# serviceberry3/weiner_slamit_v2

Measured on AMD Instinct MI355X. Metric: frames/sec ORB extract+match @640x480x8lvl, higher is better.
Workload: dtype u8; 1 GPU; BASELINE configs[1]: 640x480 8-level ORB extract (1000 features, FAST 20/7) + brute-force 256-bit Hamming best/second match vs the stream's previous frame; 256 independent streams per GPU per step; distinct_frame_pairs_per_gpu=16, parallelism=streams sharded over 1 GPU(s), no data-path collective

## Files before the change

### weiner_slamit_v2_amd/csrc/octree_table.h

```cpp
#ifndef SLAMIT_OCTREE_TABLE_H
#define SLAMIT_OCTREE_TABLE_H
#include <stdint.h>

#if defined(__HIPCC__)
#define OCT_HD __host__ __device__ __forceinline__
#else
#define OCT_HD static inline
#endif

#define OCT_FD_MAX 4

struct Box16 { short x0, y0, x1, y1; };

OCT_HD int box_quadrant(const Box16& b, int x, int y, int* mx, int* my) {
    int midx = b.x0 + ((b.x1 - b.x0 + 1) >> 1);
    int midy = b.y0 + ((b.y1 - b.y0 + 1) >> 1);
    *mx = midx; *my = midy;
    return (x < midx ? 0 : 1) + (y < midy ? 0 : 2);
}
OCT_HD Box16 child_box(const Box16& b, int q) {
    int midx = b.x0 + ((b.x1 - b.x0 + 1) >> 1);
    int midy = b.y0 + ((b.y1 - b.y0 + 1) >> 1);
    Box16 c;
    c.x0 = (q & 1) ? midx : b.x0; c.x1 = (q & 1) ? b.x1 : midx;
    c.y0 = (q & 2) ? midy : b.y0; c.y1 = (q & 2) ? b.y1 : midy;
    return c;
}

// ... 9 lines not shown
}
OCT_HD unsigned oct_rank_key(int cnt, int pos) { return ((unsigned)cnt << 12) | (unsigned)(4095 - pos); }

OCT_HD int oct_key_root(int x, float hX, int nIni) {
    const int r = (int)((float)x / hX);
    return r < nIni - 1 ? r : nIni - 1;
}
OCT_HD int oct_key_path(Box16 b, int x, int y, int FD) {
    int path = 0;
    for (int d = 0; d < FD; ++d) {
        int mx, my;
        const int q = box_quadrant(b, x, y, &mx, &my);
        b = child_box(b, q);
        path = path * 4 + q;
    }
    return path;
}

OCT_HD unsigned long long oct_pick_key(unsigned response, unsigned order) {
    return ((unsigned long long)response << 32) | (0xFFFFFFFFu - order);
}
OCT_HD unsigned oct_pick_response(unsigned long long k) { return (unsigned)(k >> 32); }
OCT_HD unsigned oct_pick_order(unsigned long long k) { return 0xFFFFFFFFu - (unsigned)k; }

OCT_HD int oct_code(int root, int depth, int path) { return (root << 16) | (depth << 12) | path; }
OCT_HD int oct_code_root(int c) { return c >> 16; }
OCT_HD int oct_code_depth(int c) { return (c >> 12) & 15; }
OCT_HD int oct_code_path(int c) { return c & 4095; }
OCT_HD int oct_code_child(int c, int q) { return oct_code(oct_code_root(c), oct_code_depth(c) + 1, 4 * oct_code_path(c) + q); }
OCT_HD int oct_child_slot(int c, int q, int HS) {
    return oct_code_root(c) * HS + oct_depth_off(oct_code_depth(c) + 1) + 4 * oct_code_path(c) + q;
}
OCT_HD int oct_node_slot(int c, int HS) { return oct_code_root(c) * HS + oct_depth_off(oct_code_depth(c)) + oct_code_path(c); }

OCT_HD bool oct_node_leaves_table(int cnt, int code, int FD) { return cnt > 1 && oct_code_depth(code) >= FD; }

OCT_HD void oct_table_sum_up(int* tab, int FD) {
    for (int d = FD - 1; d >= 1; --d)
        for (int p = 0; p < (1 << (2 * d)); ++p) {
            const int* c = &tab[oct_depth_off(d + 1) + 4 * p];
            tab[oct_depth_off(d) + p] = (c[0] + c[1]) + (c[2] + c[3]);
        }
}

#define OCT_PATH_LEFT 0x100
OCT_HD int oct_path_word(int passes, bool left) { return (passes & 0xFF) | (left ? OCT_PATH_LEFT : 0); }
// ... 93 lines not shown
```

### weiner_slamit_v2_amd/csrc/orb_api.hip

```cpp
#include <hip/hip_runtime.h>
#include <math.h>
#include <stdio.h>
#include <stdlib.h>
#include <string.h>

#include <algorithm>
#include <vector>

#include "../../include/slamit.h"
#include "orb_plan.h"
#include "slamit_internal.h"

hipError_t orbk_upload_pattern(hipStream_t st);
void orbk_resize(hipStream_t st, const uint8_t* src, int sw, int sh, size_t sstride, size_t sframe,
                 uint8_t* dst, int dw, int dh, size_t dstride, size_t dframe, const int* xofs,
                 const short* ialpha, const int* yofs, const short* ibeta, int nframes);
void orbk_resize_rows4(hipStream_t st, const uint8_t* src, size_t sstride, size_t sframe, int sh, uint8_t* dst, int dw, int dh,
                       size_t dstride, size_t dframe, const uint32_t* d_col, const uint32_t* d_row, int nframes);
void orbk_resize_rows8(hipStream_t st, const uint8_t* src, size_t sstride, size_t sframe, int sh, uint8_t* dst, int dw, int dh,
                       size_t dstride, size_t dframe, const uint32_t* d_col8, const uint32_t* d_row, int nframes);
hipError_t orbk_pyramid_bands_prepare(int smem_bytes);
void orbk_pyramid_bands(hipStream_t st, const BandTab& tab, const uint8_t* d_tables, const BandRows* d_rows, int first, int last, int nbands,
                        const uint8_t* src, size_t sstride, size_t sframe, int sh, uint8_t* pyr, size_t pyr_frame, int tile0, int smem, int nframes);
hipError_t orbk_pyramid_prepare(int smem_bytes);
void orbk_pyramid(hipStream_t st, const OrbLevel* levels, int nlevels, const PyrBox* boxes, const PyrTabs* tabs,
                  int nregions, const uint8_t* img0, size_t img0_stride, size_t img0_frame, uint8_t* pyr, int bufA_bytes,
                  int smem_bytes, int nframes, int l_first, int l_last);
hipError_t orbk_fast_prepare(int max_wcell, int max_hcell);
void orbk_fast(hipStream_t st, const FastTab& tab, int nlevels, const uint32_t* d_cells, int cells_per_frame, const uint8_t* img0,
               size_t img0_stride, size_t img0_frame, const uint8_t* pyr, unsigned long long* cand,
               size_t cand_frame_stride, int* cand_count, int iniTh, int minTh, int max_wcell, int max_hcell, int nframes);
hipError_t orbk_octree_prepare(int node_cap, int key_cap);
void orbk_octree(hipStream_t st, const OrbLevel* levels, int nlevels, const unsigned long long* cand,
                 size_t cand_frame_stride, int* cand_count, uint32_t* ws_xy, uint16_t* ws_node,
                 OrbLevelKp* lkp, size_t kp_frame_stride, int* kp_count, int node_cap, int key_cap, int nframes,
                 int level_override);
void orbk_ic_angle(hipStream_t st, const OrbLevel* levels, int nlevels, const uint8_t* img0, size_t img0_stride,
                   size_t img0_frame, const uint8_t* pyr, OrbLevelKp* lkp, size_t kp_frame_stride,
                   const int* kp_count, const KpBlockTab& tab, int nframes);
void orbk_blur_stream(hipStream_t st, const OrbLevel* levels, const uint32_t* d_inner, int n_inner, const uint32_t* d_edge, int n_edge,
                      const uint8_t* img0, size_t img0_stride, size_t img0_frame, const uint8_t* pyr, uint8_t* blur, int nframes);
void orbk_blur(hipStream_t st, const OrbLevel* levels, const uint32_t* d_tiles, int total_tiles, const uint8_t* img0,
               size_t img0_stride, size_t img0_frame, const uint8_t* pyr, uint8_t* blur, int nframes);
void orbk_describe(hipStream_t st, const OrbLevel* levels, int nlevels, const uint8_t* blur,
                   const OrbLevelKp* lkp, size_t kp_frame_stride, const int* kp_count, slamit_kp* out_kps,
                   uint8_t* out_desc, int out_cap, int* out_n, const KpBlockTab& tab, int nframes);
void orbk_pad(hipStream_t st, const uint8_t* src, int w, int h, size_t sstride, uint8_t* dst);
void orbk_decode_candidates(hipStream_t st, const OrbLevel* levels, int level, const unsigned long long* K, int n,
                            unsigned long long* order_out, int* xys);

namespace {

inline size_t round_up(size_t v, size_t a) { return (v + a - 1) / a * a; }

}

#define ORB_BLUR_SPLIT 1

struct slamit_orb {
// ... 233 lines not shown
            const OrbLevel& D = P.levels[l];
            const uint8_t* src = l == 1 ? d_gray : h->d_pyr + S.plane_off;
            size_t sstride = l == 1 ? stride : (size_t)S.stride;
            size_t sframe = l == 1 ? frame_stride : P.pyr_frame_total;
            const OrbResizeTabs& T = P.rs[l];
            orbk_resize(st, src, S.w, S.h, sstride, sframe, h->d_pyr + D.plane_off, D.w, D.h, (size_t)D.stride,
                        P.pyr_frame_total, dtab<int>(h, T.xofs_off), dtab<short>(h, T.ialpha_off), dtab<int>(h, T.yofs_off),
                        dtab<short>(h, T.ibeta_off), nframes);
        }
    }
    prof_mark(h, st, ST_RESIZE, false);
    prof_mark(h, st, ST_FAST, true);
    orbk_fast(st, P.fast, nl, dtab<uint32_t>(h, P.cells_off), (int)(P.cells.size() / 4), d_gray, stride, frame_stride, h->d_pyr, h->d_cand,
              P.cand_frame_stride, cand_count, h->p.ini_th_fast, h->p.min_th_fast, P.max_wcell, P.max_hcell, nframes);
    prof_mark(h, st, ST_FAST, false);
    if (side) {
        HIP_TRY(hipEventRecord(h->ev_pyr, st));
        HIP_TRY(hipStreamWaitEvent(h->stream_b, h->ev_pyr, 0));
        launch_blur(h->stream_b, early_done + 1, nl);
        HIP_TRY(hipEventRecord(h->ev_blur, h->stream_b));
    }
    prof_mark(h, st, ST_OCTREE, true);
    orbk_octree(st, h->d_levels, nl, h->d_cand, P.cand_frame_stride, cand_count, h->d_ws_xy, h->d_ws_node, h->d_lkp,
                P.kp_frame_stride, kp_count, P.node_cap, P.oct_key_cap, nframes, -1);
    prof_mark(h, st, ST_OCTREE, false);
    prof_mark(h, st, ST_ANGLE, true);
    orbk_ic_angle(st, h->d_levels, nl, d_gray, stride, frame_stride, h->d_pyr, h->d_lkp, P.kp_frame_stride, kp_count,
                  P.ic_blocks, nframes);
    prof_mark(h, st, ST_ANGLE, false);
    if (side) {
        HIP_TRY(hipStreamWaitEvent(st, h->ev_blur, 0));
    } else {
        prof_mark(h, st, ST_BLUR, true);
        launch_blur(st, 0, nl);
        prof_mark(h, st, ST_BLUR, false);
    }
    prof_mark(h, st, ST_DESCRIBE, true);
    orbk_describe(st, h->d_levels, nl, h->d_blur, h->d_lkp, P.kp_frame_stride, kp_count, d_kps, d_desc, cap, d_n_out,
                  P.desc_blocks, nframes);
    prof_mark(h, st, ST_DESCRIBE, false);
    ++h->prof_call;
    HIP_TRY(hipGetLastError());
    h->counters_clean = true;
    h->last_img0 = d_gray; h->last_stride = stride; h->last_frame = frame_stride; h->last_nframes = nframes;
    return SLAMIT_OK;
}

// ... 151 lines not shown
```

### weiner_slamit_v2_amd/csrc/orb_kernels.hip

```cpp
#include <hip/hip_runtime.h>
#include <stdint.h>

#include <algorithm>

#include "blur_window.h"
#include "octree_table.h"
#include "orb_types.h"
#include "slamit_math.h"
#include "wave_ops.h"
#include "../../include/slamit.h"
#include "../../include/slamit_orb_pattern.h"

#define WAVE 64

__global__ __launch_bounds__(256) void resize_level_kernel(
    const uint8_t* __restrict__ src, int sw, int sh, size_t sstride, size_t sframe,
    uint8_t* __restrict__ dst, int dw, int dh, size_t dstride, size_t dframe,
    const int* __restrict__ xofs, const short* __restrict__ ialpha,
    const int* __restrict__ yofs, const short* __restrict__ ibeta) {
    const int x4 = (blockIdx.x * 64 + (threadIdx.x & 63)) * 4;
    const int y = blockIdx.y * 4 + (threadIdx.x >> 6);
    const int f = blockIdx.z;
    if (x4 >= dw || y >= dh) return;
    const uint8_t* S = src + (size_t)f * sframe;
// ... 1081 lines not shown
    __syncthreads();
    for (int i = tid; i < n; i += NT) {
        unsigned long long b = best[i];
        unsigned order = 0xFFFFFFFFu - (unsigned)b;
        int lx = order & 63, ly = (order >> 6) & 63, cell = order >> 12;
        int ci = cell / L.nCols, cj = cell - ci * L.nCols;
        OrbLevelKp kp;
        kp.x = (int16_t)(cj * L.wCell + lx + ORB_MIN_BORDER);
        kp.y = (int16_t)(ci * L.hCell + ly + ORB_MIN_BORDER);
        kp.response = (float)(unsigned)(b >> 32);
        kp.angle = 0.f; kp.cs = 1.f; kp.sn = 0.f;
        if (i < L.kp_cap) OUT[i] = kp;
    }
    if (tid == 0) *kp_count_out = min(n, L.kp_cap);
#ifdef OCT_DIAG
    OD_STAMP(5);
    if (tid == 0) {
        const int w = blockIdx.y * gridDim.x + blockIdx.x;
        if (w < 4096) { unsigned long long* o = g_oct_ph + 8 * w; for (int k = 0; k < 6; ++k) o[k] = od_ph[k]; o[6] = ((unsigned long long)od_pass << 32) | (unsigned)n_keys; o[7] = od_rt0; o[5] = __builtin_amdgcn_s_memrealtime(); }
    }
#endif
}

template <int NT>
__device__ __forceinline__ bool octree_table_path(
    const OrbLevel& L, const unsigned long long* __restrict__ K, int n_keys, OrbLevelKp* __restrict__ OUT,
    int* __restrict__ kp_count_out, unsigned char* smem, int cap, unsigned long long* bin_best, int FD, int* s_vars, int* passes_out) {
    const int tid = threadIdx.x, lane = tid & 63;
    const int nIni = L.nIni, N = L.quota;
    const int HS = oct_table_ints(FD), NB = oct_bins(FD), leaf0 = oct_depth_off(FD);
    int* const hist = reinterpret_cast<int*>(smem);
    int* const ncode0 = reinterpret_cast<int*>(smem + (size_t)8 * cap);
    unsigned long long* const nbest = reinterpret_cast<unsigned long long*>(smem + (size_t)16 * cap);
    int* const cnt0 = reinterpret_cast<int*>(smem + (size_t)24 * cap);
    int* const elist = cnt0 + 2 * cap;
    unsigned* const ekey = reinterpret_cast<unsigned*>(elist + cap);
    int* const scanbuf = elist + 4 * cap;
    int* const rankv = scanbuf + 5 * cap;
    int* const sorted = rankv + cap;
    Box16* const rootbox = reinterpret_cast<Box16*>(scanbuf);
    OD_DECL;

    if (tid < nIni) { Box16 b; b.x0 = (short)L.rootUL[tid]; b.y0 = 0; b.x1 = (short)L.rootUR[tid]; b.y1 = (short)L.boxH; rootbox[tid] = b; }
    for (int e = tid; e < nIni * HS; e += NT) hist[e] = 0;
    for (int e = tid; e < nIni * NB; e += NT) bin_best[e] = 0ull;
    __syncthreads();
    {
        const int nCols = L.nCols, wCell = L.wCell, hCell = L.hCell;
        const unsigned inv_cols = 0xFFFFFFFFu / (unsigned)nCols + 1u;
        const float hX = L.hX;
        for (int kb4 = 0; kb4 < n_keys; kb4 += 4 * NT) {
            unsigned long long c4[4];
#pragma unroll
            for (int j = 0; j < 4; ++j) c4[j] = K[min(kb4 + j * NT + tid, n_keys - 1)];
#pragma unroll
            for (int j = 0; j < 4; ++j) {
                const int kb = kb4 + j * NT;
                if (kb >= n_keys) break;
                const bool valid = kb + tid < n_keys;
                const unsigned order = (unsigned)c4[j];
                const int lx = order & 63, ly = (order >> 6) & 63, cell = order >> 12;
                const int ci = (int)__umulhi((unsigned)cell, inv_cols), cj = cell - ci * nCols;
                const int x = cj * wCell + lx, y = ci * hCell + ly;
                const int r = oct_key_root(x, hX, nIni);
                const int path = oct_key_path(rootbox[r], x, y, FD);
                const int bin = valid ? r * NB + path : -1;
                const int prev = __shfl_up(bin, 1);
                const bool head = lane == 0 || bin != prev;
                const unsigned long long heads = __ballot(head);
                const unsigned long long rest = (heads >> lane) >> 1;
                const int last = rest ? lane + (int)__builtin_ctzll(rest) : 63;
                unsigned long long pk = valid ? oct_pick_key((unsigned)(c4[j] >> 32), order) : 0ull;
#pragma unroll
                for (int s = 1; s < 64; s <<= 1) {
                    const unsigned long long o = __shfl_down(pk, s);
                    pk = (lane + s <= last && o > pk) ? o : pk;
                }
                if (head && bin >= 0) {
                    atomicAdd(&hist[r * HS + leaf0 + path], last - lane + 1);
                    atomicMax(&bin_best[bin], pk);
                }
            }
        }
    }
    __syncthreads();
    OD_STAMP(0);

    if (tid < 64) {
        for (int d = FD - 1; d >= 1; --d) {
            const int per = 1 << (2 * d), off = oct_depth_off(d), offc = oct_depth_off(d + 1);
            for (int e = lane; e < nIni * per; e += 64) {
                const int r = e >> (2 * d), pth = e & (per - 1);
                const int* c = &hist[r * HS + offc + 4 * pth];
                hist[r * HS + off + pth] = (c[0] + c[1]) + (c[2] + c[3]);
            }
            wave_mem_sync();
        }
        if (lane == 0) {
            int m = 0;
            for (int i = 0; i < nIni; ++i) {
                const int c = (hist[i * HS] + hist[i * HS + 1]) + (hist[i * HS + 2] + hist[i * HS + 3]);
                if (c > 0) { cnt0[m] = c; ncode0[m] = oct_code(i, 0, 0); ++m; }
            }
            s_vars[0] = m;
        }
        wave_mem_sync();
// ... 95 lines not shown
            else if (!careful && n + nToExpand * 3 > N) careful = true;
        }
        if (!left) {
            int* const rootlab = scanbuf;
            int* const lab = scanbuf + ORB_MAX_ROOTS;
            for (int e = lane; e < nIni * HS; e += 64) lab[e] = -1;
            if (lane < ORB_MAX_ROOTS) rootlab[lane] = -1;
            for (int i = lane; i < n; i += 64) nbest[i] = 0ull;
            wave_mem_sync();
            for (int i = lane; i < n; i += 64) {
                const int c = ncode0[cur * cap + i];
                if (oct_code_depth(c) == 0) rootlab[oct_code_root(c)] = i;
                else lab[oct_node_slot(c, HS)] = i;
            }
        }
        if (lane == 0) { s_vars[0] = n; s_vars[2] = passes; s_vars[3] = left; }
    }
    __syncthreads();
    OD_STAMP(1);
    *passes_out = s_vars[2];
    if (s_vars[3]) return false;
    const int n = s_vars[0];

    {
        const int* rootlab = scanbuf;
        const int* lab = scanbuf + ORB_MAX_ROOTS;
        for (int b = tid; b < nIni * NB; b += NT) {
            const int r = b >> (2 * FD), pth = b & (NB - 1);
            if (hist[r * HS + leaf0 + pth] <= 0) continue;
            int node = rootlab[r];
            for (int d = 1; d <= FD; ++d) {
                const int v = lab[r * HS + oct_depth_off(d) + (pth >> (2 * (FD - d)))];
                node = v >= 0 ? v : node;
            }
            if (node >= 0) atomicMax(&nbest[node], bin_best[b]);
        }
    }
    __syncthreads();
    for (int i = tid; i < n; i += NT) {
        const unsigned long long b = nbest[i];
        const unsigned order = oct_pick_order(b);
        int lx = order & 63, ly = (order >> 6) & 63, cell = order >> 12;
        int ci = cell / L.nCols, cj = cell - ci * L.nCols;
        OrbLevelKp kp;
        kp.x = (int16_t)(cj * L.wCell + lx + ORB_MIN_BORDER);
        kp.y = (int16_t)(ci * L.hCell + ly + ORB_MIN_BORDER);
        kp.response = (float)oct_pick_response(b);
        kp.angle = 0.f; kp.cs = 1.f; kp.sn = 0.f;
        if (i < L.kp_cap) OUT[i] = kp;
    }
    if (tid == 0) *kp_count_out = min(n, L.kp_cap);
#ifdef OCT_DIAG
    OD_STAMP(2);
    if (tid == 0) {
        const int w = blockIdx.y * gridDim.x + blockIdx.x;
        if (w < 4096) { unsigned long long* o = g_oct_ph + 8 * w; for (int k = 0; k < 5; ++k) o[k] = od_ph[k]; o[6] = ((unsigned long long)s_vars[2] << 32) | (unsigned)n_keys; o[7] = od_rt0; o[5] = __builtin_amdgcn_s_memrealtime(); }
    }
#endif
    return true;
}

template <int OCT_NT>
__global__ __launch_bounds__(OCT_NT) void octree_kernel(
    const OrbLevel* __restrict__ levels, int nlevels,
    const unsigned long long* __restrict__ cand, size_t cand_frame_stride,
    int* __restrict__ cand_count,
    uint32_t* __restrict__ ws_xy, uint16_t* __restrict__ ws_node,
    OrbLevelKp* __restrict__ lkp, size_t kp_frame_stride, int* __restrict__ kp_count,
    int node_cap, int key_cap, int level_override ) {
    extern __shared__ __attribute__((aligned(16))) unsigned char smem[];
    __shared__ int wave_tmp[OCT_NT / 64];
    __shared__ int s_vars[4];
    uint32_t* k_xy = reinterpret_cast<uint32_t*>(smem + orbk_octree_node_bytes(node_cap));
    uint16_t* k_nd = reinterpret_cast<uint16_t*>(k_xy + key_cap);
    const int level = level_override >= 0 ? level_override : blockIdx.y;
    const int frame = blockIdx.x;
    const OrbLevel& L = levels[level];
    const int kidx = frame * nlevels + level;
    const int n_raw = cand_count[kidx * ORB_CC_PAD];
    const int n_keys = min(n_raw, L.cand_cap);
    __syncthreads();
    if (threadIdx.x == 0) { cand_count[kidx * ORB_CC_PAD] = 0; cand_count[kidx * ORB_CC_PAD + 1] = n_raw; }
    const unsigned long long* K = cand + L.cand_off + (size_t)frame * cand_frame_stride;
    OrbLevelKp* OUT = lkp + L.kp_off + (size_t)frame * kp_frame_stride;
    if (n_keys == 0) {
        if (threadIdx.x == 0) { kp_count[kidx] = 0; cand_count[kidx * ORB_CC_PAD + 2] = oct_path_word(0, false); }
        return;
    }
    const int FD = nIniFD(L.nIni, 2 * node_cap);
    int table_passes = 0;
    bool done = false;
    if (oct_table_fits(L.nIni, FD, (long)key_cap * 6, n_keys))
        done = octree_table_path<OCT_NT>(L, K, n_keys, OUT, &kp_count[kidx], smem, node_cap, reinterpret_cast<unsigned long long*>(k_xy), FD,
                                         s_vars, &table_passes);
    if (threadIdx.x == 0) cand_count[kidx * ORB_CC_PAD + 2] = oct_path_word(table_passes, !done);
    if (done) return;
    if (n_keys <= key_cap)
        octree_body<OCT_NT, true>(L, K, n_keys, k_xy, k_nd, OUT, &kp_count[kidx], smem, node_cap, wave_tmp, s_vars);
    else
        octree_body<OCT_NT, false>(L, K, n_keys, ws_xy + L.cand_off + (size_t)frame * cand_frame_stride,
                                        ws_node + L.cand_off + (size_t)frame * cand_frame_stride, OUT, &kp_count[kidx], smem,
                                        node_cap, wave_tmp, s_vars);
}

struct DiscTable { signed char uv[64][32]; int n; };
__constant__ DiscTable c_disc;

static DiscTable make_disc() {
    static const int umax[16] = {15, 15, 15, 15, 14, 14, 14, 13, 13, 12, 11, 10, 9, 8, 6, 3};
    DiscTable t;
    for (int l = 0; l < 64; ++l) for (int k = 0; k < 32; ++k) t.uv[l][k] = 0;
    t.n = 0;
    for (int v = -15; v <= 15; ++v)
        for (int u = -umax[v < 0 ? -v : v]; u <= umax[v < 0 ? -v : v]; ++u) {
            t.uv[t.n & 63][2 * (t.n >> 6)] = (signed char)u; t.uv[t.n & 63][2 * (t.n >> 6) + 1] = (signed char)v;
            ++t.n;
        }
// ... 630 lines not shown
                           (unsigned)img0_stride, img0_frame, pyr, cand, cand_frame_stride, cand_count, iniTh, minTh, tile_rows,
                           sc_rows, kp_cap, xcd_frames);
    else
        hipLaunchKernelGGL(fast_cells_kernel<FAST_PL>, grid, dim3(64 * wpb), smem, st, tab, reinterpret_cast<const uint4*>(d_cells), nlevels, cells_per_frame, img0,
                           (unsigned)img0_stride, img0_frame, pyr, cand, cand_frame_stride, cand_count, iniTh, minTh, tile_rows,
                           sc_rows, kp_cap, xcd_frames);
}

hipError_t orbk_octree_prepare(int node_cap, int key_cap) {
    static int prepared = 0;
    const int want = (int)orbk_octree_smem(node_cap, key_cap);
    if (want <= prepared) return hipSuccess;
    prepared = want;
    hipError_t e = hipFuncSetAttribute(reinterpret_cast<const void*>(octree_kernel<256>), hipFuncAttributeMaxDynamicSharedMemorySize, want);
    if (e != hipSuccess) return e;
    e = hipFuncSetAttribute(reinterpret_cast<const void*>(octree_kernel<OCT_THREADS>), hipFuncAttributeMaxDynamicSharedMemorySize, want);
    if (e != hipSuccess) return e;
    return hipFuncSetAttribute(reinterpret_cast<const void*>(octree_kernel<1024>), hipFuncAttributeMaxDynamicSharedMemorySize, want);
}

void orbk_octree(hipStream_t st, const OrbLevel* levels, int nlevels, const unsigned long long* cand,
                 size_t cand_frame_stride, int* cand_count, uint32_t* ws_xy, uint16_t* ws_node,
                 OrbLevelKp* lkp, size_t kp_frame_stride, int* kp_count, int node_cap, int key_cap, int nframes,
                 int level_override) {
    dim3 grid(nframes, level_override >= 0 ? 1 : nlevels);
    const int nt = nframes >= 96 ? 256 : nframes <= 16 ? 1024 : OCT_THREADS;
    if (nframes >= 96) key_cap = std::min(key_cap, OCT_BIG_BATCH_KEYS);
    if (nt == 1024)
        hipLaunchKernelGGL(octree_kernel<1024>, grid, dim3(1024), orbk_octree_smem(node_cap, key_cap), st, levels, nlevels, cand,
                           cand_frame_stride, cand_count, ws_xy, ws_node, lkp, kp_frame_stride, kp_count, node_cap,
                           key_cap, level_override);
    else if (nt == 256)
        hipLaunchKernelGGL(octree_kernel<256>, grid, dim3(256), orbk_octree_smem(node_cap, key_cap), st, levels, nlevels, cand,
                           cand_frame_stride, cand_count, ws_xy, ws_node, lkp, kp_frame_stride, kp_count, node_cap,
                           key_cap, level_override);
    else
        hipLaunchKernelGGL(octree_kernel<OCT_THREADS>, grid, dim3(OCT_THREADS), orbk_octree_smem(node_cap, key_cap), st, levels, nlevels, cand,
                           cand_frame_stride, cand_count, ws_xy, ws_node, lkp, kp_frame_stride, kp_count, node_cap,
                           key_cap, level_override);
}

void orbk_ic_angle(hipStream_t st, const OrbLevel* levels, int nlevels, const uint8_t* img0,
                   size_t img0_stride, size_t img0_frame, const uint8_t* pyr, OrbLevelKp* lkp,
                   size_t kp_frame_stride, const int* kp_count, const KpBlockTab& tab, int nframes) {
    const unsigned per_frame = tab.first[ORB_MAX_LEVELS];
    if (!per_frame) return;
    if (nframes >= 16)
        hipLaunchKernelGGL(ic_angle_kernel, dim3((unsigned)(((nframes + 7) / 8) * 8) * per_frame), dim3(256), 0, st, levels,
                           nlevels, img0, img0_stride, img0_frame, pyr, lkp, kp_frame_stride, kp_count, nframes, tab);
    else
        hipLaunchKernelGGL(ic_angle_kernel, dim3(per_frame, nframes), dim3(256), 0, st, levels,
                           nlevels, img0, img0_stride, img0_frame, pyr, lkp, kp_frame_stride, kp_count, 0, tab);
}

void orbk_blur_stream(hipStream_t st, const OrbLevel* levels, const uint32_t* d_inner, int n_inner, const uint32_t* d_edge, int n_edge,
                      const uint8_t* img0, size_t img0_stride, size_t img0_frame, const uint8_t* pyr, uint8_t* blur, int nframes) {
    const int wgs = (std::max(n_inner, 0) + 15) / 16 + (std::max(n_edge, 0) + 15) / 16;
    if (wgs <= 0) return;
    hipLaunchKernelGGL(blur_stream_kernel, dim3(wgs, nframes), dim3(256), 0, st, levels, reinterpret_cast<const uint4*>(d_inner), (unsigned)std::max(n_inner, 0),
                       reinterpret_cast<const uint4*>(d_edge), (unsigned)std::max(n_edge, 0), img0, img0_stride, img0_frame, pyr, blur);
}

// ... 36 lines not shown
```

### weiner_slamit_v2_amd/csrc/orb_plan.cc

```cpp
#include "orb_plan.h"

#include <math.h>
#include <string.h>

#include <algorithm>

namespace {

inline int cv_round(double v) { return (int)lrint(v); }
inline size_t round_up(size_t v, size_t a) { return (v + a - 1) / a * a; }

inline short sat_short(float v) {
    int iv = cv_round((double)v);
    return (short)(iv < -32768 ? -32768 : iv > 32767 ? 32767 : iv);
}

void plan_scales(const slamit_orb_params& p, OrbPlan& P) {
    const int nl = p.nlevels;
    const double scaleFactor = (double)p.scale_factor;
    P.scale.assign(nl, 1.f); P.sigma2.assign(nl, 1.f); P.inv_scale.assign(nl, 1.f); P.inv_sigma2.assign(nl, 1.f);
    for (int i = 1; i < nl; ++i) {
        P.scale[i] = (float)(P.scale[i - 1] * scaleFactor);
        P.sigma2[i] = P.scale[i] * P.scale[i];
    }
    for (int i = 0; i < nl; ++i) { P.inv_scale[i] = 1.0f / P.scale[i]; P.inv_sigma2[i] = 1.0f / P.sigma2[i]; }
    P.per_level.assign(nl, 0);
    float factor = (float)(1.0f / scaleFactor);
    float nDesired = p.nfeatures * (1 - factor) / (1 - (float)pow((double)factor, (double)nl));
// ... 69 lines not shown

void fast_cells(OrbPlan& P) {
    auto magic = [](int g) { return (uint32_t)((1u << 20) / (unsigned)std::max(g, 1) + 1u); };
    for (int l = 0; l < (int)P.levels.size(); ++l) {
        const OrbLevel& L = P.levels[l];
        for (int c = 0; c < L.ncells; ++c) {
            const int ci = c / L.nCols, cj = c - ci * L.nCols;
            const int iniX = ORB_MIN_BORDER + cj * L.wCell, iniY = ORB_MIN_BORDER + ci * L.hCell;
            if (iniY >= L.maxBorderY - 3 || iniX >= L.maxBorderX - 6) continue;
            const int cw = std::min(L.wCell + 6, L.maxBorderX - iniX), ch = std::min(L.hCell + 6, L.maxBorderY - iniY);
            const int sw = cw - 6, sh = ch - 6;
            if (sw <= 0 || sh <= 0) continue;
            const uint32_t w[4] = {(uint32_t)l | ((uint32_t)c << 8), (uint32_t)iniX | ((uint32_t)iniY << 16),
                                   (uint32_t)cw | ((uint32_t)ch << 8), magic((sw + 3) >> 2)};
            P.cells.insert(P.cells.end(), w, w + 4);
        }
        FastLevel& D = P.fast.lv[l];
        D.cell_base = L.cell_base; D.nCols = L.nCols; D.wCell = L.wCell; D.hCell = L.hCell;
        D.maxBorderX = L.maxBorderX; D.maxBorderY = L.maxBorderY; D.stride = L.stride; D.cand_cap = L.cand_cap;
        D.plane_off = L.plane_off; D.plane_bytes = L.plane_bytes; D.cand_off = L.cand_off;
    }
}

void blur_strips(OrbPlan& P) {
    const int nl = (int)P.levels.size();
    for (int l = 0; l < nl; ++l) {
        OrbLevel& L = P.levels[l];
        L.blur_tile_base = (int)(P.blur_all.tab.size() / 4);
        for (int by = 0; by < L.h; by += ORB_BLUR_STRIP_H)
            for (int bx = 0; bx < L.w; bx += 64) {
                const uint32_t t[4] = {(uint32_t)l, (uint32_t)bx, (uint32_t)by, 0u};
                const bool inside = bx >= 4 && bx + 68 <= L.w && (L.stride & 3) == 0;
                for (OrbStrips* S : {&P.blur_all, inside ? &P.blur_str : &P.blur_edge}) S->tab.insert(S->tab.end(), t, t + 4);
            }
        for (OrbStrips* S : {&P.blur_all, &P.blur_str, &P.blur_edge}) S->base[l + 1] = (int)(S->tab.size() / 4);
    }
}

void resize_axis(int dn, int sn, bool clampx, std::vector<int32_t>& ofs, std::vector<int16_t>& coef) {
    double inv_scale = (double)dn / sn;
    double scale = 1. / inv_scale;
    ofs.resize(dn);
    coef.resize(2 * (size_t)dn);
    for (int d = 0; d < dn; ++d) {
        float f = (float)((d + 0.5) * scale - 0.5);
        int s = (int)floor(f);
// ... 166 lines not shown
    }
    P.bands.swap(segs);
}

void plan_table_block(OrbPlan& P) {
    size_t off = 0;
    auto take = [&](size_t bytes) { const size_t at = round_up(off, 256); off = at + bytes; return at; };
    const int nl = (int)P.levels.size();
    P.levels_off = take(sizeof(OrbLevel) * nl);
    P.cells_off = take(sizeof(uint32_t) * P.cells.size());
    for (OrbStrips* S : {&P.blur_all, &P.blur_str, &P.blur_edge}) S->off = take(sizeof(uint32_t) * S->tab.size());
    for (int l = 1; l < nl; ++l) {
        OrbResizeTabs& T = P.rs[l];
        T.xofs_off = take(sizeof(int32_t) * T.xofs.size()); T.ialpha_off = take(sizeof(int16_t) * T.ialpha.size());
        T.yofs_off = take(sizeof(int32_t) * T.yofs.size()); T.ibeta_off = take(sizeof(int16_t) * T.ibeta.size());
        T.col4_off = take(sizeof(uint32_t) * T.col4.size()); T.row4_off = take(sizeof(uint32_t) * T.row4.size());
        T.col8_off = take(sizeof(uint32_t) * T.col8.size());
    }
    P.boxes_off = take(sizeof(PyrBox) * P.boxes.size());
    P.tabs_off = take(P.pyr_regions ? sizeof(PyrTabs) * nl : 0);
    for (OrbBandSeg& G : P.bands) G.rows_off = take(sizeof(BandRows) * G.rows.size());
    if (!P.bands.empty())
        for (int l = 1; l < nl; ++l) { P.band_tab.lv[l].col_off = P.rs[l].col8_off; P.band_tab.lv[l].row_off = P.rs[l].row4_off; }
    P.table_bytes = round_up(off, 256);
}

}

bool orb_plan(const slamit_orb_params& p, const OrbPlanOptions& o, OrbPlan& plan, const char** why) {
    plan = OrbPlan();
    OrbPlan& P = plan;
    P.node_cap = 8; P.max_kp_level = 1;
    P.rows4_ok = true;
    plan_scales(p, P);
    P.max_out = p.nfeatures + 3 * p.nlevels;
    const bool empty = p.width == 0 || p.height == 0;
    if (!empty && !plan_levels(p, P, why)) return false;
    P.oct_key_cap = octree_key_cap(P.node_cap, p.width, p.height);
    if (orbk_octree_smem(P.node_cap, P.oct_key_cap) > 160 * 1024 - 1024 || P.node_cap >= 4096) {
        *why = "slamit_orb_create: nfeatures too large for the LDS octree";
        return false;
    }
    if (!orb_plan_kp_blocks(P.levels, ORB_IC_KP_PER_WG, P.ic_blocks) || !orb_plan_kp_blocks(P.levels, ORB_DESC_KP_PER_WG, P.desc_blocks)) {
        *why = "slamit_orb_create: nfeatures too large for the keypoint passes";
        return false;
    }
    fast_cells(P);
    blur_strips(P);
    plan_resize(o, P);
    plan_pyramid_boxes(p, P);
    plan_bands(P);
    plan_table_block(P);
    return true;
}

bool orb_plan_kp_blocks(const std::vector<OrbLevel>& levels, int per, KpBlockTab& tab) {
    const int nl = (int)levels.size();
    if (nl > ORB_MAX_LEVELS || per < 1) return false;
    long at = 0;
    for (int l = 0; l <= ORB_MAX_LEVELS; ++l) {
        if (at > 65535) return false;
        tab.first[l] = (uint16_t)at;
        if (l < nl) at += (std::max(levels[l].kp_cap, 0) + per - 1) / per;
    }
    return true;
}

bool orb_plan_band_segment(const OrbPlan& P, int first, int last, int nbands, size_t lds_budget, OrbBandSeg& seg) {
    const int nl = (int)P.levels.size(), nlv = last - first;
    if (first < 0 || last >= nl || nlv < 1 || nbands < 1) return false;
    seg = OrbBandSeg();
// ... 19 lines not shown
                t = std::max(t, (size_t)(cmp1 - cmp0) * band_pitch(P.levels[l].w) + ORB_BAND_SLACK);
            }
        }
    }
    seg.tile0 = (int)round_up(tile[0], 16);
    seg.smem = seg.tile0 + (int)round_up(tile[1], 16);
    return (size_t)seg.smem <= lds_budget;
}

void orb_plan_image(const OrbPlan& P, const uint8_t* base, std::vector<uint8_t>& img) {
    img.assign(P.table_bytes, 0);
    auto put = [&](size_t off, const void* src, size_t bytes) { if (bytes) memcpy(img.data() + off, src, bytes); };
    auto put_vec = [&](size_t off, const auto& v) { put(off, v.data(), sizeof(v[0]) * v.size()); };
    put(P.levels_off, P.levels.data(), sizeof(OrbLevel) * P.levels.size());
    put_vec(P.cells_off, P.cells);
    for (const OrbStrips* S : {&P.blur_all, &P.blur_str, &P.blur_edge}) put_vec(S->off, S->tab);
    for (size_t l = 1; l < P.rs.size(); ++l) {
        const OrbResizeTabs& T = P.rs[l];
        put_vec(T.xofs_off, T.xofs); put_vec(T.ialpha_off, T.ialpha); put_vec(T.yofs_off, T.yofs); put_vec(T.ibeta_off, T.ibeta);
        put_vec(T.col4_off, T.col4); put_vec(T.row4_off, T.row4); put_vec(T.col8_off, T.col8);
    }
    put_vec(P.boxes_off, P.boxes);
    for (const OrbBandSeg& G : P.bands) put_vec(G.rows_off, G.rows);
    if (!P.pyr_regions) return;
    std::vector<PyrTabs> tabs(P.levels.size(), PyrTabs{nullptr, nullptr, nullptr, nullptr});
    auto at = [&](size_t off) { return (uintptr_t)base + off; };
    for (size_t l = 1; l < tabs.size(); ++l) {
        const OrbResizeTabs& T = P.rs[l];
        tabs[l].xofs = reinterpret_cast<const int32_t*>(at(T.xofs_off)); tabs[l].ialpha = reinterpret_cast<const int16_t*>(at(T.ialpha_off));
        tabs[l].yofs = reinterpret_cast<const int32_t*>(at(T.yofs_off)); tabs[l].ibeta = reinterpret_cast<const int16_t*>(at(T.ibeta_off));
    }
    put_vec(P.tabs_off, tabs);
}
```

### weiner_slamit_v2_amd/csrc/orb_plan.h

```cpp
#ifndef SLAMIT_ORB_PLAN_H
#define SLAMIT_ORB_PLAN_H

#include <stddef.h>
#include <stdint.h>

#include <vector>

#include "../../include/slamit.h"
#include "orb_types.h"

struct OrbPlanOptions {
    bool resize_no8;
};

struct OrbStrips {
    std::vector<uint32_t> tab;
    int base[ORB_MAX_LEVELS + 1];
    size_t off;
};

struct OrbResizeTabs {
    std::vector<int32_t> xofs, yofs;
    std::vector<int16_t> ialpha, ibeta;
    std::vector<uint32_t> col4, row4;
    std::vector<uint32_t> col8;
    size_t xofs_off, ialpha_off, yofs_off, ibeta_off, col4_off, row4_off, col8_off;
};

struct OrbBandSeg {
    int first, last, nbands;
    std::vector<BandRows> rows;
    int tile0, smem;
    size_t rows_off;
};

struct OrbPlan {
    std::vector<float> scale, inv_scale, sigma2, inv_sigma2;
    std::vector<int> per_level;
    std::vector<OrbLevel> levels;
    size_t pyr_frame_total, blur_frame_total, cand_frame_stride, kp_frame_stride;
    int max_out, node_cap, oct_key_cap, max_kp_level, max_wcell, max_hcell;
    std::vector<uint32_t> cells;
    size_t cells_off;
    FastTab fast;
    KpBlockTab ic_blocks, desc_blocks;
    OrbStrips blur_all, blur_str, blur_edge;
    std::vector<OrbResizeTabs> rs;
    bool rows4_ok;
    int pyr_regions, pyr_bufA, pyr_smem;
    std::vector<PyrBox> boxes;
    size_t levels_off, boxes_off, tabs_off;
    std::vector<OrbBandSeg> bands;
    BandTab band_tab;
    size_t table_bytes;
};

bool orb_plan(const slamit_orb_params& p, const OrbPlanOptions& o, OrbPlan& plan, const char** why);

bool orb_plan_kp_blocks(const std::vector<OrbLevel>& levels, int per, KpBlockTab& tab);

bool orb_plan_band_segment(const OrbPlan& plan, int first, int last, int nbands, size_t lds_budget, OrbBandSeg& seg);

void orb_plan_image(const OrbPlan& plan, const uint8_t* base, std::vector<uint8_t>& img);

#endif
```

### weiner_slamit_v2_amd/csrc/orb_types.h

```cpp
#ifndef SLAMIT_ORB_TYPES_H
#define SLAMIT_ORB_TYPES_H

#include <stddef.h>
#include <stdint.h>

#ifdef __HIPCC__
#define ORB_HD __host__ __device__
#else
#define ORB_HD
#endif

#define ORB_MAX_LEVELS 16
#define ORB_MAX_ROOTS 8
#define ORB_MIN_BORDER 16
#define ORB_CELL_MAX 59
#define ORB_TILE_MAX (ORB_CELL_MAX + 6)
#define ORB_CC_PAD 32
#define BLUR_STEPS 4
#define ORB_BLUR_STRIP_H (16 * BLUR_STEPS)

ORB_HD inline size_t orbk_octree_node_bytes(int node_cap) {
    return ((size_t)node_cap * (8 + 2 * 8 + 2 * 4 + 4 * 4 + 5 * 4 + 4 + 4) + 64 + 15) & ~(size_t)15;
}
ORB_HD inline size_t orbk_octree_smem(int node_cap, int key_cap) { return orbk_octree_node_bytes(node_cap) + (size_t)key_cap * 6; }
// ... 11 lines not shown
    uint64_t blur_bytes;
    int32_t nCols, nRows, wCell, hCell;
    int32_t maxBorderX, maxBorderY;
    int32_t cell_base;
    int32_t ncells;
    int32_t blur_tile_base;
    uint64_t cand_off;
    int32_t cand_cap;
    int32_t nIni;
    float hX;
    int32_t rootUL[ORB_MAX_ROOTS], rootUR[ORB_MAX_ROOTS];
    int32_t boxH;
    int32_t kp_off, kp_cap;
    float scale;
    float patch_size;
};

struct FastLevel {
    int32_t cell_base, nCols, wCell, hCell, maxBorderX, maxBorderY, stride, cand_cap;
    uint64_t plane_off, plane_bytes, cand_off;
};
struct FastTab { FastLevel lv[ORB_MAX_LEVELS]; };

struct PyrBox {
    int16_t ox0, oy0, ox1, oy1;
    int16_t nx0, ny0, nx1, ny1;
};
struct PyrTabs {
    const int32_t* xofs; const int16_t* ialpha;
    const int32_t* yofs; const int16_t* ibeta;
};

struct BandLevel {
    uint64_t col_off, row_off;
    uint64_t plane_off;
    int32_t ngroups, dstride, pitch;
    uint32_t inv_groups;
};
struct BandTab { BandLevel lv[ORB_MAX_LEVELS]; };
struct BandRows { uint16_t own0, own1, cmp0, cmp1; };
#define ORB_BAND_LDS_BUDGET (78 * 1024)
#define ORB_BAND_SLACK 16

#define ORB_IC_KP_PER_WG 32
#define ORB_DESC_KP_PER_WG 16
struct alignas(4) KpBlockTab { uint16_t first[ORB_MAX_LEVELS + 1]; };
// ... 10 lines not shown
```

Measured before the change: 354,500 frames/s.

## Precompute octree bin lookup tables and use 32-bit pick keys with DPP reductions

The octree histogram sweep no longer computes each key's root and quadtree path per candidate. It reads per-level x/y bin tables that are built on the host at plan time and staged into LDS, with the x and y path bits interleaved so the bin is a single add. When the cell count fits, pick keys shrink from 64 to 32 bits (8-bit response, 24-bit order). The wave segmented max now uses DPP row ops within 16-lane groups instead of 64-lane shuffles. The aim is to cut ALU, LDS and atomic cost in the octree stage, at the price of extra table memory, more template variants, and a 32-bit key that assumes responses fit in 8 bits.

New measurement: 355,800 frames/s, median of 6. No clear change (+0.4%).

```diff
diff --git a/weiner_slamit_v2_amd/csrc/octree_table.h b/weiner_slamit_v2_amd/csrc/octree_table.h
--- a/weiner_slamit_v2_amd/csrc/octree_table.h
+++ b/weiner_slamit_v2_amd/csrc/octree_table.h
@@ -3,7 +3,7 @@
 #include <stdint.h>
 
 #if defined(__HIPCC__)
-#define OCT_HD __host__ __device__ __forceinline__
+#define OCT_HD __host__ __device__ inline __attribute__((always_inline))
 #else
 #define OCT_HD static inline
 #endif
@@ -59,6 +59,28 @@
 }
 OCT_HD unsigned oct_pick_response(unsigned long long k) { return (unsigned)(k >> 32); }
 OCT_HD unsigned oct_pick_order(unsigned long long k) { return 0xFFFFFFFFu - (unsigned)k; }
+
+#define OCT_PICK32_CELLS 4096
+OCT_HD bool oct_pick32_fits(int ncells) { return ncells <= OCT_PICK32_CELLS; }
+OCT_HD unsigned oct_pick_key32(unsigned response, unsigned order) { return (response << 24) | (0xFFFFFFu - order); }
+OCT_HD unsigned oct_pick_response32(unsigned k) { return k >> 24; }
+OCT_HD unsigned oct_pick_order32(unsigned k) { return 0xFFFFFFu - (k & 0xFFFFFFu); }
+
+OCT_HD bool oct_bin_tables_fit(int nIni, int FD) { return FD > 0 && (long)nIni * oct_bins(FD) <= 65536; }
+OCT_HD int oct_bin_table_len(int ncell, int cell_size) { return (ncell * cell_size + 64 + 1) & ~1; }
+OCT_HD Box16 oct_root_box(int ul, int ur, int boxH) { Box16 b; b.x0 = (short)ul; b.y0 = 0; b.x1 = (short)ur; b.y1 = (short)boxH; return b; }
+OCT_HD void oct_bin_tables(int nIni, float hX, const int* rootUL, const int* rootUR, int boxH, int FD, int nx, int ny,
+                           uint16_t* xtab, uint16_t* ytab) {
+    const int NB = oct_bins(FD);
+    for (int x = 0; x < nx; ++x) {
+        const int r = oct_key_root(x, hX, nIni);
+        xtab[x] = (uint16_t)(r * NB + (oct_key_path(oct_root_box(rootUL[r], rootUR[r], boxH), x, 0, FD) & 0x5555));
+    }
+    for (int y = 0; y < ny; ++y) ytab[y] = (uint16_t)(oct_key_path(oct_root_box(rootUL[0], rootUR[0], boxH), 0, y, FD) & 0xAAAA);
+}
+OCT_HD bool oct_bin_tables_in_lds(int nIni, int FD, int pick_bytes, int nx, int ny, long key_bytes) {
+    return nx > 0 && (long)nIni * pick_bytes * oct_bins(FD) + 2L * (nx + ny) <= key_bytes;
+}
 
 OCT_HD int oct_code(int root, int depth, int path) { return (root << 16) | (depth << 12) | path; }
 OCT_HD int oct_code_root(int c) { return c >> 16; }
diff --git a/weiner_slamit_v2_amd/csrc/orb_api.hip b/weiner_slamit_v2_amd/csrc/orb_api.hip
--- a/weiner_slamit_v2_amd/csrc/orb_api.hip
+++ b/weiner_slamit_v2_amd/csrc/orb_api.hip
@@ -34,7 +34,7 @@
 void orbk_octree(hipStream_t st, const OrbLevel* levels, int nlevels, const unsigned long long* cand,
                  size_t cand_frame_stride, int* cand_count, uint32_t* ws_xy, uint16_t* ws_node,
                  OrbLevelKp* lkp, size_t kp_frame_stride, int* kp_count, int node_cap, int key_cap, int nframes,
-                 int level_override);
+                 int level_override, const OctBinTab& bins, const uint8_t* d_tables);
 void orbk_ic_angle(hipStream_t st, const OrbLevel* levels, int nlevels, const uint8_t* img0, size_t img0_stride,
                    size_t img0_frame, const uint8_t* pyr, OrbLevelKp* lkp, size_t kp_frame_stride,
                    const int* kp_count, const KpBlockTab& tab, int nframes);
@@ -314,7 +314,7 @@
     }
     prof_mark(h, st, ST_OCTREE, true);
     orbk_octree(st, h->d_levels, nl, h->d_cand, P.cand_frame_stride, cand_count, h->d_ws_xy, h->d_ws_node, h->d_lkp,
-                P.kp_frame_stride, kp_count, P.node_cap, P.oct_key_cap, nframes, -1);
+                P.kp_frame_stride, kp_count, P.node_cap, P.oct_key_cap, nframes, -1, P.oct_tab, h->d_tables);
     prof_mark(h, st, ST_OCTREE, false);
     prof_mark(h, st, ST_ANGLE, true);
     orbk_ic_angle(st, h->d_levels, nl, d_gray, stride, frame_stride, h->d_pyr, h->d_lkp, P.kp_frame_stride, kp_count,
diff --git a/weiner_slamit_v2_amd/csrc/orb_kernels.hip b/weiner_slamit_v2_amd/csrc/orb_kernels.hip
--- a/weiner_slamit_v2_amd/csrc/orb_kernels.hip
+++ b/weiner_slamit_v2_amd/csrc/orb_kernels.hip
@@ -1127,13 +1127,123 @@
 #endif
 }
 
+template <typename PK> struct OctPick;
+template <> struct OctPick<unsigned long long> {
+    static __device__ __forceinline__ unsigned long long key(unsigned response, unsigned order) { return oct_pick_key(response, order); }
+    static __device__ __forceinline__ unsigned order(unsigned long long k) { return oct_pick_order(k); }
+    static __device__ __forceinline__ unsigned response(unsigned long long k) { return oct_pick_response(k); }
+};
+template <> struct OctPick<uint32_t> {
+    static __device__ __forceinline__ uint32_t key(unsigned response, unsigned order) { return oct_pick_key32(response, order); }
+    static __device__ __forceinline__ unsigned order(uint32_t k) { return oct_pick_order32(k); }
+    static __device__ __forceinline__ unsigned response(uint32_t k) { return oct_pick_response32(k); }
+};
+
+template <int NT, typename PK, bool TAB>
+__device__ __forceinline__ void octree_table_sweep(
+    const OrbLevel& L, const unsigned long long* __restrict__ K, int n_keys, int* hist, PK* bin_best, Box16* rootbox,
+    const uint32_t* __restrict__ g_tab, int nx, int ny, int FD) {
+    const int tid = threadIdx.x, lane = tid & 63;
+    const int nIni = L.nIni;
+    const int HS = oct_table_ints(FD), NB = oct_bins(FD), leaf0 = oct_depth_off(FD);
+    uint16_t* const xtab = reinterpret_cast<uint16_t*>(bin_best + nIni * NB);
+    uint16_t* const ytab = xtab + nx;
+    unsigned long long c4[4];
+#pragma unroll
+    for (int j = 0; j < 4; ++j) c4[j] = K[min(j * NT + tid, n_keys - 1)];
+    if (TAB) {
+        uint32_t* const t32 = reinterpret_cast<uint32_t*>(xtab);
+        for (int e = tid; e < (nx + ny) >> 1; e += NT) t32[e] = g_tab[e];
+    } else if (tid < nIni) rootbox[tid] = oct_root_box(L.rootUL[tid], L.rootUR[tid], L.boxH);
+    for (int e = tid; e < nIni * HS; e += NT) hist[e] = 0;
+    for (int e = tid; e < nIni * NB; e += NT) bin_best[e] = 0;
+    __syncthreads();
+    const int nCols = L.nCols, wCell = L.wCell, hCell = L.hCell;
+    const unsigned inv_cols = 0xFFFFFFFFu / (unsigned)nCols + 1u;
+    const float hX = L.hX;
+    const int lane32 = lane & 31;
+    for (int kb4 = 0; kb4 < n_keys; kb4 += 4 * NT) {
+        if (kb4 > 0) {
+#pragma unroll
+            for (int j = 0; j < 4; ++j) c4[j] = K[min(kb4 + j * NT + tid, n_keys - 1)];
+        }
+#pragma unroll
+        for (int j = 0; j < 4; ++j) {
+            const int kb = kb4 + j * NT;
+            if (kb >= n_keys) break;
+            const bool valid = kb + tid < n_keys;
+            const unsigned order = (unsigned)c4[j];
+            const unsigned lx = order & 63, ly = (order >> 6) & 63, cell = order >> 12;
+            const unsigned ci = __umulhi(cell, inv_cols), cj = cell - __umul24(ci, (unsigned)nCols);
+            const int x = (int)(__umul24(cj, (unsigned)wCell) + lx), y = (int)(__umul24(ci, (unsigned)hCell) + ly);
+            int b;
+            if (TAB) b = (int)xtab[x] + (int)ytab[y];
+            else {
+                const int r = oct_key_root(x, hX, nIni);
+                b = r * NB + oct_key_path(rootbox[r], x, y, FD);
+            }
+            const int bin = valid ? b : -1;
+            const int prev = __builtin_amdgcn_update_dpp(-2, bin, 0x111, 0xF, 0xF, false);
+            const bool head = bin != prev;
+            const unsigned long long heads = __ballot(head);
+            const unsigned rest = ((lane < 32 ? (unsigned)heads : (unsigned)(heads >> 32)) >> lane32) >> 1;
+            const int room = rest ? (int)__builtin_ctz(rest) : 31 - lane32;
+            PK pk = valid ? OctPick<PK>::key((unsigned)(c4[j] >> 32), order) : (PK)0;
+            PK o;
+            o = dpp<0x101>(pk); pk = (room >= 1 && o > pk) ? o : pk;
+            o = dpp<0x102>(pk); pk = (room >= 2 && o > pk) ? o : pk;
+            o = dpp<0x104>(pk); pk = (room >= 4 && o > pk) ? o : pk;
+            o = dpp<0x108>(pk); pk = (room >= 8 && o > pk) ? o : pk;
+            if (head && bin >= 0) {
+                atomicAdd(&hist[bin + ((bin >> (2 * FD)) + 1) * leaf0], room + 1);
+                atomicMax(&bin_best[bin], pk);
+            }
+        }
+    }
+}
+
+template <int NT, typename PK>
+__device__ __forceinline__ void octree_table_picks(
+    const OrbLevel& L, OrbLevelKp* __restrict__ OUT, const int* hist, const PK* bin_best, PK* nbest, const int* rootlab, const int* lab,
+    int n, int FD) {
+    const int tid = threadIdx.x;
+    const int nIni = L.nIni;
+    const int HS = oct_table_ints(FD), NB = oct_bins(FD), leaf0 = oct_depth_off(FD);
+    for (int b = tid; b < nIni * NB; b += NT) {
+        const int r = b >> (2 * FD), pth = b & (NB - 1);
+        if (hist[r * HS + leaf0 + pth] <= 0) continue;
+        int node = rootlab[r];
+        for (int d = 1; d <= FD; ++d) {
+            const int v = lab[r * HS + oct_depth_off(d) + (pth >> (2 * (FD - d)))];
+            node = v >= 0 ? v : node;
+        }
+        if (node >= 0) atomicMax(&nbest[node], bin_best[b]);
+    }
+    __syncthreads();
+    const int nCols = L.nCols;
+    const unsigned inv_cols = 0xFFFFFFFFu / (unsigned)nCols + 1u;
+    for (int i = tid; i < n; i += NT) {
+        const PK b = nbest[i];
+        const unsigned order = OctPick<PK>::order(b);
+        const int lx = order & 63, ly = (order >> 6) & 63, cell = order >> 12;
+        const int ci = (int)__umulhi((unsigned)cell, inv_cols), cj = cell - ci * nCols;
+        OrbLevelKp kp;
+        kp.x = (int16_t)(cj * L.wCell + lx + ORB_MIN_BORDER);
+        kp.y = (int16_t)(ci * L.hCell + ly + ORB_MIN_BORDER);
+        kp.response = (float)OctPick<PK>::response(b);
+        kp.angle = 0.f; kp.cs = 1.f; kp.sn = 0.f;
+        if (i < L.kp_cap) OUT[i] = kp;
+    }
+}
+
 template <int NT>
 __device__ __forceinline__ bool octree_table_path(
     const OrbLevel& L, const unsigned long long* __restrict__ K, int n_keys, OrbLevelKp* __restrict__ OUT,
-    int* __restrict__ kp_count_out, unsigned char* smem, int cap, unsigned long long* bin_best, int FD, int* s_vars, int* passes_out) {
+    int* __restrict__ kp_count_out, unsigned char* smem, int cap, unsigned long long* bin_best, long key_bytes,
+    const uint32_t* __restrict__ g_tab, int nx, int ny, int FD, int* s_vars, int* passes_out) {
     const int tid = threadIdx.x, lane = tid & 63;
     const int nIni = L.nIni, N = L.quota;
-    const int HS = oct_table_ints(FD), NB = oct_bins(FD), leaf0 = oct_depth_off(FD);
+    const int HS = oct_table_ints(FD);
     int* const hist = reinterpret_cast<int*>(smem);
     int* const ncode0 = reinterpret_cast<int*>(smem + (size_t)8 * cap);
     unsigned long long* const nbest = reinterpret_cast<unsigned long long*>(smem + (size_t)16 * cap);
@@ -1146,47 +1256,14 @@
     Box16* const rootbox = reinterpret_cast<Box16*>(scanbuf);
     OD_DECL;
 
-    if (tid < nIni) { Box16 b; b.x0 = (short)L.rootUL[tid]; b.y0 = 0; b.x1 = (short)L.rootUR[tid]; b.y1 = (short)L.boxH; rootbox[tid] = b; }
-    for (int e = tid; e < nIni * HS; e += NT) hist[e] = 0;
-    for (int e = tid; e < nIni * NB; e += NT) bin_best[e] = 0ull;
-    __syncthreads();
-    {
-        const int nCols = L.nCols, wCell = L.wCell, hCell = L.hCell;
-        const unsigned inv_cols = 0xFFFFFFFFu / (unsigned)nCols + 1u;
-        const float hX = L.hX;
-        for (int kb4 = 0; kb4 < n_keys; kb4 += 4 * NT) {
-            unsigned long long c4[4];
-#pragma unroll
-            for (int j = 0; j < 4; ++j) c4[j] = K[min(kb4 + j * NT + tid, n_keys - 1)];
-#pragma unroll
-            for (int j = 0; j < 4; ++j) {
-                const int kb = kb4 + j * NT;
-                if (kb >= n_keys) break;
-                const bool valid = kb + tid < n_keys;
-                const unsigned order = (unsigned)c4[j];
-                const int lx = order & 63, ly = (order >> 6) & 63, cell = order >> 12;
-                const int ci = (int)__umulhi((unsigned)cell, inv_cols), cj = cell - ci * nCols;
-                const int x = cj * wCell + lx, y = ci * hCell + ly;
-                const int r = oct_key_root(x, hX, nIni);
-                const int path = oct_key_path(rootbox[r], x, y, FD);
-                const int bin = valid ? r * NB + path : -1;
-                const int prev = __shfl_up(bin, 1);
-                const bool head = lane == 0 || bin != prev;
-                const unsigned long long heads = __ballot(head);
-                const unsigned long long rest = (heads >> lane) >> 1;
-                const int last = rest ? lane + (int)__builtin_ctzll(rest) : 63;
-                unsigned long long pk = valid ? oct_pick_key((unsigned)(c4[j] >> 32), order) : 0ull;
-#pragma unroll
-                for (int s = 1; s < 64; s <<= 1) {
-                    const unsigned long long o = __shfl_down(pk, s);
-                    pk = (lane + s <= last && o > pk) ? o : pk;
-                }
-                if (head && bin >= 0) {
-                    atomicAdd(&hist[r * HS + leaf0 + path], last - lane + 1);
-                    atomicMax(&bin_best[bin], pk);
-                }
-            }
-        }
+    const bool k32 = oct_pick32_fits(L.ncells);
+    const bool tab = oct_bin_tables_in_lds(nIni, FD, k32 ? 4 : 8, nx, ny, key_bytes);
+    if (k32) {
+        if (tab) octree_table_sweep<NT, uint32_t, true>(L, K, n_keys, hist, reinterpret_cast<uint32_t*>(bin_best), rootbox, g_tab, nx, ny, FD);
+        else octree_table_sweep<NT, uint32_t, false>(L, K, n_keys, hist, reinterpret_cast<uint32_t*>(bin_best), rootbox, g_tab, nx, ny, FD);
+    } else {
+        if (tab) octree_table_sweep<NT, unsigned long long, true>(L, K, n_keys, hist, bin_best, rootbox, g_tab, nx, ny, FD);
+        else octree_table_sweep<NT, unsigned long long, false>(L, K, n_keys, hist, bin_best, rootbox, g_tab, nx, ny, FD);
     }
     __syncthreads();
     OD_STAMP(0);
@@ -1328,33 +1405,8 @@
     if (s_vars[3]) return false;
     const int n = s_vars[0];
 
-    {
-        const int* rootlab = scanbuf;
-        const int* lab = scanbuf + ORB_MAX_ROOTS;
-        for (int b = tid; b < nIni * NB; b += NT) {
-            const int r = b >> (2 * FD), pth = b & (NB - 1);
-            if (hist[r * HS + leaf0 + pth] <= 0) continue;
-            int node = rootlab[r];
-            for (int d = 1; d <= FD; ++d) {
-                const int v = lab[r * HS + oct_depth_off(d) + (pth >> (2 * (FD - d)))];
-                node = v >= 0 ? v : node;
-            }
-            if (node >= 0) atomicMax(&nbest[node], bin_best[b]);
-        }
-    }
-    __syncthreads();
-    for (int i = tid; i < n; i += NT) {
-        const unsigned long long b = nbest[i];
-        const unsigned order = oct_pick_order(b);
-        int lx = order & 63, ly = (order >> 6) & 63, cell = order >> 12;
-        int ci = cell / L.nCols, cj = cell - ci * L.nCols;
-        OrbLevelKp kp;
-        kp.x = (int16_t)(cj * L.wCell + lx + ORB_MIN_BORDER);
-        kp.y = (int16_t)(ci * L.hCell + ly + ORB_MIN_BORDER);
-        kp.response = (float)oct_pick_response(b);
-        kp.angle = 0.f; kp.cs = 1.f; kp.sn = 0.f;
-        if (i < L.kp_cap) OUT[i] = kp;
-    }
+    if (k32) octree_table_picks<NT, uint32_t>(L, OUT, hist, reinterpret_cast<const uint32_t*>(bin_best), reinterpret_cast<uint32_t*>(nbest), scanbuf, scanbuf + ORB_MAX_ROOTS, n, FD);
+    else octree_table_picks<NT, unsigned long long>(L, OUT, hist, bin_best, nbest, scanbuf, scanbuf + ORB_MAX_ROOTS, n, FD);
     if (tid == 0) *kp_count_out = min(n, L.kp_cap);
 #ifdef OCT_DIAG
     OD_STAMP(2);
@@ -1373,7 +1425,7 @@
     int* __restrict__ cand_count,
     uint32_t* __restrict__ ws_xy, uint16_t* __restrict__ ws_node,
     OrbLevelKp* __restrict__ lkp, size_t kp_frame_stride, int* __restrict__ kp_count,
-    int node_cap, int key_cap, int level_override ) {
+    int node_cap, int key_cap, int level_override , const OctBinTab bins, const uint8_t* __restrict__ tables) {
     extern __shared__ __attribute__((aligned(16))) unsigned char smem[];
     __shared__ int wave_tmp[OCT_NT / 64];
     __shared__ int s_vars[4];
@@ -1397,8 +1449,9 @@
     int table_passes = 0;
     bool done = false;
     if (oct_table_fits(L.nIni, FD, (long)key_cap * 6, n_keys))
-        done = octree_table_path<OCT_NT>(L, K, n_keys, OUT, &kp_count[kidx], smem, node_cap, reinterpret_cast<unsigned long long*>(k_xy), FD,
-                                         s_vars, &table_passes);
+        done = octree_table_path<OCT_NT>(L, K, n_keys, OUT, &kp_count[kidx], smem, node_cap, reinterpret_cast<unsigned long long*>(k_xy),
+                                         (long)key_cap * 6, reinterpret_cast<const uint32_t*>(tables + bins.lv[level].off), bins.lv[level].nx,
+                                         bins.lv[level].ny, FD, s_vars, &table_passes);
     if (threadIdx.x == 0) cand_count[kidx * ORB_CC_PAD + 2] = oct_path_word(table_passes, !done);
     if (done) return;
     if (n_keys <= key_cap)
@@ -2075,22 +2128,22 @@
 void orbk_octree(hipStream_t st, const OrbLevel* levels, int nlevels, const unsigned long long* cand,
                  size_t cand_frame_stride, int* cand_count, uint32_t* ws_xy, uint16_t* ws_node,
                  OrbLevelKp* lkp, size_t kp_frame_stride, int* kp_count, int node_cap, int key_cap, int nframes,
-                 int level_override) {
+                 int level_override, const OctBinTab& bins, const uint8_t* d_tables) {
     dim3 grid(nframes, level_override >= 0 ? 1 : nlevels);
     const int nt = nframes >= 96 ? 256 : nframes <= 16 ? 1024 : OCT_THREADS;
     if (nframes >= 96) key_cap = std::min(key_cap, OCT_BIG_BATCH_KEYS);
     if (nt == 1024)
         hipLaunchKernelGGL(octree_kernel<1024>, grid, dim3(1024), orbk_octree_smem(node_cap, key_cap), st, levels, nlevels, cand,
                            cand_frame_stride, cand_count, ws_xy, ws_node, lkp, kp_frame_stride, kp_count, node_cap,
-                           key_cap, level_override);
+                           key_cap, level_override, bins, d_tables);
     else if (nt == 256)
         hipLaunchKernelGGL(octree_kernel<256>, grid, dim3(256), orbk_octree_smem(node_cap, key_cap), st, levels, nlevels, cand,
                            cand_frame_stride, cand_count, ws_xy, ws_node, lkp, kp_frame_stride, kp_count, node_cap,
-                           key_cap, level_override);
+                           key_cap, level_override, bins, d_tables);
     else
         hipLaunchKernelGGL(octree_kernel<OCT_THREADS>, grid, dim3(OCT_THREADS), orbk_octree_smem(node_cap, key_cap), st, levels, nlevels, cand,
                            cand_frame_stride, cand_count, ws_xy, ws_node, lkp, kp_frame_stride, kp_count, node_cap,
-                           key_cap, level_override);
+                           key_cap, level_override, bins, d_tables);
 }
 
 void orbk_ic_angle(hipStream_t st, const OrbLevel* levels, int nlevels, const uint8_t* img0,
diff --git a/weiner_slamit_v2_amd/csrc/orb_plan.cc b/weiner_slamit_v2_amd/csrc/orb_plan.cc
--- a/weiner_slamit_v2_amd/csrc/orb_plan.cc
+++ b/weiner_slamit_v2_amd/csrc/orb_plan.cc
@@ -4,6 +4,8 @@
 #include <string.h>
 
 #include <algorithm>
+
+#include "octree_table.h"
 
 namespace {
 
@@ -119,6 +121,21 @@
     }
 }
 
+void octree_bin_tables(OrbPlan& P) {
+    const int nl = (int)P.levels.size();
+    P.oct_bins.assign(nl, std::vector<uint16_t>());
+    for (int l = 0; l < nl; ++l) {
+        const OrbLevel& L = P.levels[l];
+        const int FD = nIniFD(L.nIni, 2 * P.node_cap);
+        if (!oct_bin_tables_fit(L.nIni, FD)) continue;
+        const int nx = oct_bin_table_len(L.nCols, L.wCell), ny = oct_bin_table_len(L.nRows, L.hCell);
+        if (nx > 65535 || ny > 65535) continue;
+        P.oct_bins[l].resize((size_t)nx + ny);
+        oct_bin_tables(L.nIni, L.hX, L.rootUL, L.rootUR, L.boxH, FD, nx, ny, P.oct_bins[l].data(), P.oct_bins[l].data() + nx);
+        P.oct_tab.lv[l].nx = (uint16_t)nx; P.oct_tab.lv[l].ny = (uint16_t)ny;
+    }
+}
+
 void blur_strips(OrbPlan& P) {
     const int nl = (int)P.levels.size();
     for (int l = 0; l < nl; ++l) {
@@ -331,6 +348,7 @@
     for (OrbBandSeg& G : P.bands) G.rows_off = take(sizeof(BandRows) * G.rows.size());
     if (!P.bands.empty())
         for (int l = 1; l < nl; ++l) { P.band_tab.lv[l].col_off = P.rs[l].col8_off; P.band_tab.lv[l].row_off = P.rs[l].row4_off; }
+    for (int l = 0; l < nl; ++l) P.oct_tab.lv[l].off = (uint32_t)take(sizeof(uint16_t) * P.oct_bins[l].size());
     P.table_bytes = round_up(off, 256);
 }
 
@@ -356,6 +374,7 @@
     }
     fast_cells(P);
     blur_strips(P);
+    if (!empty) octree_bin_tables(P);
     plan_resize(o, P);
     plan_pyramid_boxes(p, P);
     plan_bands(P);
@@ -421,6 +440,7 @@
     }
     put_vec(P.boxes_off, P.boxes);
     for (const OrbBandSeg& G : P.bands) put_vec(G.rows_off, G.rows);
+    for (size_t l = 0; l < P.oct_bins.size(); ++l) put_vec(P.oct_tab.lv[l].off, P.oct_bins[l]);
     if (!P.pyr_regions) return;
     std::vector<PyrTabs> tabs(P.levels.size(), PyrTabs{nullptr, nullptr, nullptr, nullptr});
     auto at = [&](size_t off) { return (uintptr_t)base + off; };
diff --git a/weiner_slamit_v2_amd/csrc/orb_plan.h b/weiner_slamit_v2_amd/csrc/orb_plan.h
--- a/weiner_slamit_v2_amd/csrc/orb_plan.h
+++ b/weiner_slamit_v2_amd/csrc/orb_plan.h
@@ -44,6 +44,8 @@
     size_t cells_off;
     FastTab fast;
     KpBlockTab ic_blocks, desc_blocks;
+    std::vector<std::vector<uint16_t>> oct_bins;
+    OctBinTab oct_tab;
     OrbStrips blur_all, blur_str, blur_edge;
     std::vector<OrbResizeTabs> rs;
     bool rows4_ok;
diff --git a/weiner_slamit_v2_amd/csrc/orb_types.h b/weiner_slamit_v2_amd/csrc/orb_types.h
--- a/weiner_slamit_v2_amd/csrc/orb_types.h
+++ b/weiner_slamit_v2_amd/csrc/orb_types.h
@@ -57,6 +57,9 @@
 };
 struct FastTab { FastLevel lv[ORB_MAX_LEVELS]; };
 
+struct OctBinLevel { uint32_t off; uint16_t nx, ny; };
+struct OctBinTab { OctBinLevel lv[ORB_MAX_LEVELS]; };
+
 struct PyrBox {
     int16_t ox0, oy0, ox1, oy1;
     int16_t nx0, ny0, nx1, ny1;
```
